# ShahzaibAhmad05/NextSearch-api

Measured on AMD Instinct MI355X. Metric: queries/sec at k=10 over 1M-doc index; achieved HBM GB/s vs peak, higher is better.
Workload: dtype f32

## Files before the change

nextsearch-api_amd/csrc/ns_api.hip:

```cpp
#include <hip/hip_runtime.h>

#include <algorithm>
#include <cmath>
#include <cstdarg>
#include <cstdio>
#include <cstdlib>
#include <cstring>
#include <string>
#include <vector>

#include "../../include/nextsearch_hip.h"
#include "ns_internal.h"
#include "ns_plan.hpp"
#include "ns_kernels.hip"
#include "ns_wave_kernel.hip"
#include "ns_driver_kernel.hip"
#include "ns_prune_kernel.hip"
#include "ns_merge_kernel.hip"
#include "ns_tile_kernel.hip"
#include "ns_invert.hip"
#include "ns_ingest.hip"
#include "ns_sem.hip"
#include "ns_suggest.hip"

// ... 1838 lines not shown
    ns_ctx* ctx = nullptr;
    uint32_t rows = 0, dim = 0, rows_pad = 0;
    float* d_vt = nullptr;
};

extern "C" int ns_sem_upload(ns_ctx* ctx, const float* vecs, uint32_t n_rows, uint32_t dim, ns_sem** out) {
    if (!ctx) return fail(nullptr, NS_E_INVAL, "ns_sem_upload: ctx is NULL");
    if (!out || !vecs || !n_rows || !dim) return fail(ctx, NS_E_INVAL, "ns_sem_upload: empty table or null argument");
    *out = nullptr;
    HIPCHK(ctx, hipSetDevice(ctx->device));
    ns_sem* s = new ns_sem();
    s->ctx = ctx; s->rows = n_rows; s->dim = dim; s->rows_pad = (n_rows + 63u) & ~63u;
    float* d_in = nullptr;
    hipError_t e = hipMalloc((void**)&s->d_vt, (size_t)dim * s->rows_pad * 4);
    if (e == hipSuccess) e = hipMalloc((void**)&d_in, (size_t)n_rows * dim * 4);
    if (e == hipSuccess) e = hipMemcpyAsync(d_in, vecs, (size_t)n_rows * dim * 4, hipMemcpyHostToDevice, ctx->stream);
    if (e == hipSuccess) {
        hipLaunchKernelGGL(k_sem_transpose, dim3((s->rows_pad + 31) / 32, (dim + 31) / 32), dim3(256), 0, ctx->stream, d_in, s->d_vt, n_rows, dim, s->rows_pad);
        e = hipGetLastError();
    }
    if (e == hipSuccess) e = hipStreamSynchronize(ctx->stream);
    (void)hipFree(d_in);
    if (e != hipSuccess) {
        (void)hipFree(s->d_vt);
        delete s;
        return fail(ctx, e == hipErrorOutOfMemory ? NS_E_NOMEM : NS_E_HIP, "ns_sem_upload: %s", hipGetErrorString(e));
    }
    *out = s;
    return NS_OK;
}

extern "C" int ns_sem_release(ns_ctx* ctx, ns_sem* sem) {
    if (!ctx || !sem || sem->ctx != ctx) return fail(ctx, NS_E_INVAL, "ns_sem_release: table does not belong to this ctx");
    HIPCHK(ctx, hipSetDevice(ctx->device));
    HIPCHK(ctx, hipStreamSynchronize(ctx->stream));
    (void)hipFree(sem->d_vt);
    delete sem;
    return NS_OK;
}

extern "C" int ns_sem_topk(ns_ctx* ctx, ns_sem* sem, const float* qvecs, uint32_t n_q, uint32_t topk, float min_sim,
                           const uint32_t* ban_off, const uint32_t* ban_rows, uint32_t* rows_out, float* sims_out,
                           uint32_t* counts_out, float* device_ms_out) {
    if (!ctx || !sem || sem->ctx != ctx) return fail(ctx, NS_E_INVAL, "ns_sem_topk: table does not belong to this ctx");
    if (topk < 1 || topk > (uint32_t)kSemMaxK) return fail(ctx, NS_E_INVAL, "ns_sem_topk: topk=%u outside [1,%d]", topk, kSemMaxK);
    if (device_ms_out) *device_ms_out = 0.0f;
    if (!n_q) return NS_OK;
    if (!qvecs || !rows_out || !sims_out || !counts_out) return fail(ctx, NS_E_INVAL, "ns_sem_topk: null argument");
    HIPCHK(ctx, hipSetDevice(ctx->device));
    hipStream_t st = ctx->stream;
    const uint32_t dim = sem->dim, rows = sem->rows, rp = sem->rows_pad;
    const uint32_t cap = ((rows + 63) / 64) * topk;
    const uint32_t n_groups = (n_q + kSemB - 1) / kSemB;
    const uint32_t n_ban = ban_off ? ban_off[n_q] : 0;
    std::vector<uint32_t> goff((size_t)n_groups * (kSemB + 1), 0), grows(std::max<uint32_t>(n_ban, 1), 0);
    if (n_ban && !ban_rows) return fail(ctx, NS_E_INVAL, "ns_sem_topk: ban_rows is NULL");
    if (n_ban) std::memcpy(grows.data(), ban_rows, (size_t)n_ban * 4);
    for (uint32_t g = 0; g < n_groups; g++)
        for (uint32_t b = 0; b <= (uint32_t)kSemB; b++) {
            const uint32_t qi = std::min(g * kSemB + b, n_q);
            goff[(size_t)g * (kSemB + 1) + b] = ban_off ? ban_off[qi] : 0;
        }
    std::vector<float> qpad((size_t)n_groups * kSemB * dim, 0.0f);
    std::memcpy(qpad.data(), qvecs, (size_t)n_q * dim * 4);

    float *d_q = nullptr, *d_osims = nullptr;
    uint32_t *d_goff = nullptr, *d_grows = nullptr, *d_orows = nullptr, *d_ocnt = nullptr, *d_count = nullptr;
    uint64_t* d_cand = nullptr;
    hipEvent_t ev0 = nullptr, ev1 = nullptr;
    hipError_t e = hipSuccess;
    auto chk = [&](hipError_t r) { if (e == hipSuccess) e = r; };
    const size_t n_pad = (size_t)n_groups * kSemB;
    size_t off = 0;
    auto place = [&](size_t bytes) { const size_t o = off; off = (off + std::max<size_t>(bytes, 1) + 255) & ~(size_t)255; return o; };
    const size_t o_q = place(qpad.size() * 4), o_cand = place((size_t)kSemB * cap * 8), o_goff = place(goff.size() * 4), o_count = place((size_t)kSemB * 4),
                 o_grows = place(grows.size() * 4), o_orows = place(n_pad * topk * 4), o_osims = place(n_pad * topk * 4), o_ocnt = place(n_pad * 4);
    const size_t block_bytes = off;
    char* blk = nullptr;
    chk(pool_alloc(ctx, (void**)&blk, block_bytes));
    if (e == hipSuccess) {
        d_q = (float*)(blk + o_q); d_cand = (uint64_t*)(blk + o_cand); d_goff = (uint32_t*)(blk + o_goff); d_count = (uint32_t*)(blk + o_count);
        d_grows = (uint32_t*)(blk + o_grows); d_orows = (uint32_t*)(blk + o_orows); d_osims = (float*)(blk + o_osims); d_ocnt = (uint32_t*)(blk + o_ocnt);
    }
    chk(hipEventCreate(&ev0));
    chk(hipEventCreate(&ev1));
    if (e == hipSuccess) {
        chk(hipMemcpyAsync(d_q, qpad.data(), qpad.size() * 4, hipMemcpyHostToDevice, st));
        chk(hipMemcpyAsync(d_goff, goff.data(), goff.size() * 4, hipMemcpyHostToDevice, st));
        chk(hipMemcpyAsync(d_grows, grows.data(), grows.size() * 4, hipMemcpyHostToDevice, st));
        chk(hipMemsetAsync(d_count, 0, (size_t)kSemB * 4, st));
        chk(hipEventRecord(ev0, st));
        for (uint32_t g = 0; g < n_groups; g++) {
            hipLaunchKernelGGL(k_sem_scan_topk, dim3((rows + 255) / 256), dim3(256), 0, st, sem->d_vt, rows, rp, dim, d_q + (size_t)g * kSemB * dim, min_sim,
                               d_goff + (size_t)g * (kSemB + 1), d_grows, topk, cap, d_cand, d_count);
            hipLaunchKernelGGL(k_sem_final_topk, dim3(kSemB), dim3(256), 0, st, d_cand, cap, d_count, topk, d_orows + (size_t)g * kSemB * topk, d_osims + (size_t)g * kSemB * topk, d_ocnt + (size_t)g * kSemB);
        }
        chk(hipEventRecord(ev1, st));
        chk(hipGetLastError());
        chk(hipMemcpyAsync(rows_out, d_orows, (size_t)n_q * topk * 4, hipMemcpyDeviceToHost, st));
        chk(hipMemcpyAsync(sims_out, d_osims, (size_t)n_q * topk * 4, hipMemcpyDeviceToHost, st));
        chk(hipMemcpyAsync(counts_out, d_ocnt, (size_t)n_q * 4, hipMemcpyDeviceToHost, st));
        chk(hipStreamSynchronize(st));
        float ms = 0.0f;
        if (e == hipSuccess && device_ms_out && hipEventElapsedTime(&ms, ev0, ev1) == hipSuccess) *device_ms_out = ms;
    }
    if (blk) { (void)hipStreamSynchronize(st); pool_free(ctx, blk, block_bytes); }
    if (ev0) (void)hipEventDestroy(ev0);
    if (ev1) (void)hipEventDestroy(ev1);
    if (e != hipSuccess) return fail(ctx, e == hipErrorOutOfMemory ? NS_E_NOMEM : NS_E_HIP, "ns_sem_topk: %s", hipGetErrorString(e));
    return NS_OK;
}

struct ns_ac {
    ns_ctx* ctx = nullptr;
    uint32_t n = 0;
    AcLevels lv{};
    uint8_t* d_pool = nullptr;
    uint32_t* d_offs = nullptr;
    uint64_t* d_heads = nullptr;
    uint64_t* d_keys = nullptr;
    uint64_t* d_tree = nullptr;
};

static void ac_free(ns_ac* ac) {
    if (!ac) return;
    (void)hipFree(ac->d_pool);
    (void)hipFree(ac->d_offs);
    (void)hipFree(ac->d_heads);
    (void)hipFree(ac->d_keys);
    (void)hipFree(ac->d_tree);
    delete ac;
}
static void ac_free_fwd(ns_ac* ac) { ac_free(ac); }

extern "C" int ns_ac_upload(ns_ctx* ctx, const uint8_t* pool, const uint64_t* offsets, const uint32_t* scores, uint32_t n_terms, ns_ac** out) {
    if (!ctx) return fail(nullptr, NS_E_INVAL, "ns_ac_upload: ctx is NULL");
    if (!out) return fail(ctx, NS_E_INVAL, "ns_ac_upload: out is NULL");
    *out = nullptr;
    if (n_terms && (!offsets || !scores)) return fail(ctx, NS_E_INVAL, "ns_ac_upload: null argument");
    if (n_terms == ~0u) return fail(ctx, NS_E_INVAL, "ns_ac_upload: %u terms (the index ~0 is reserved)", n_terms);
    const uint64_t pool_bytes = n_terms ? offsets[n_terms] : 0;
    if (n_terms && offsets[0] != 0) return fail(ctx, NS_E_INVAL, "ns_ac_upload: offsets[0] = %llu, not 0", (unsigned long long)offsets[0]);
    if (pool_bytes >= (1ull << 32)) return fail(ctx, NS_E_INVAL, "ns_ac_upload: a pool of %llu bytes (>= 4 GiB)", (unsigned long long)pool_bytes);
    if (pool_bytes && !pool) return fail(ctx, NS_E_INVAL, "ns_ac_upload: pool is NULL");
    for (uint32_t i = 0; i < n_terms; i++) {
        if (offsets[i + 1] < offsets[i]) return fail(ctx, NS_E_INVAL, "ns_ac_upload: offsets decrease at term %u", i);
        if (i == 0) continue;
        const uint64_t la = offsets[i] - offsets[i - 1], lb = offsets[i + 1] - offsets[i];
        const int c = std::memcmp(pool + offsets[i - 1], pool + offsets[i], (size_t)std::min(la, lb));
        if (c > 0 || (c == 0 && la > lb)) return fail(ctx, NS_E_INVAL, "ns_ac_upload: terms %u and %u are not in byte order", i - 1, i);
    }
    HIPCHK(ctx, hipSetDevice(ctx->device));
    ns_ac* ac = new ns_ac();
    ac->ctx = ctx;
    ac->n = n_terms;
    if (n_terms == 0) {
        ctx->acs.push_back(ac);
        *out = ac;
        return NS_OK;
    }
    std::vector<uint32_t> offs32(n_terms + 1);
    std::vector<uint64_t> heads(n_terms), keys(n_terms);
    for (uint32_t i = 0; i <= n_terms; i++) offs32[i] = (uint32_t)offsets[i];
    for (uint32_t i = 0; i < n_terms; i++) {
        const uint64_t len = offsets[i + 1] - offsets[i];
        uint64_t h = 0;
        for (uint64_t j = 0; j < len && j < 8; j++) h |= (uint64_t)pool[offsets[i] + j] << (56 - 8 * j);
        heads[i] = h;
        keys[i] = ((uint64_t)(~scores[i]) << 32) | i;
    }
    uint32_t nodes = (n_terms + kAcFan - 1) / kAcFan;
    uint64_t tree_keys = 0;
    for (;;) {
        ac->lv.off[ac->lv.n_levels] = tree_keys;
        ac->lv.nodes[ac->lv.n_levels] = nodes;
        tree_keys += (uint64_t)nodes * kAcTop;
        ac->lv.n_levels++;
        if (nodes <= (uint32_t)kAcFan) break;
        nodes = (nodes + kAcFan - 1) / kAcFan;
    }
    hipStream_t st = ctx->stream;
    hipError_t e = hipSuccess;
    auto chk = [&](hipError_t r) { if (e == hipSuccess) e = r; };
    chk(hipMalloc((void**)&ac->d_pool, std::max<uint64_t>(pool_bytes, 1)));
    chk(hipMalloc((void**)&ac->d_offs, (size_t)(n_terms + 1) * 4));
    chk(hipMalloc((void**)&ac->d_heads, (size_t)n_terms * 8));
    chk(hipMalloc((void**)&ac->d_keys, (size_t)n_terms * 8));
    chk(hipMalloc((void**)&ac->d_tree, (size_t)tree_keys * 8));
    if (e == hipSuccess) {
        if (pool_bytes) chk(hipMemcpyAsync(ac->d_pool, pool, pool_bytes, hipMemcpyHostToDevice, st));
        chk(hipMemcpyAsync(ac->d_offs, offs32.data(), offs32.size() * 4, hipMemcpyHostToDevice, st));
        chk(hipMemcpyAsync(ac->d_heads, heads.data(), heads.size() * 8, hipMemcpyHostToDevice, st));
        chk(hipMemcpyAsync(ac->d_keys, keys.data(), keys.size() * 8, hipMemcpyHostToDevice, st));
    }
    for (uint32_t j = 0; j < ac->lv.n_levels && e == hipSuccess; j++) {
        const uint64_t* src = j == 0 ? ac->d_keys : ac->d_tree + ac->lv.off[j - 1];
        const uint32_t n_src = j == 0 ? n_terms : ac->lv.nodes[j - 1];
        hipLaunchKernelGGL(k_ac_build, dim3((ac->lv.nodes[j] + 3) / 4), dim3(256), 0, st, src, n_src, j == 0 ? 1u : (uint32_t)kAcTop,
                           j == 0 ? 1u : (uint32_t)kAcTop, ac->d_tree + ac->lv.off[j], ac->lv.nodes[j]);
        chk(hipGetLastError());
    }
    chk(hipStreamSynchronize(st));
    if (e != hipSuccess) {
        ac_free(ac);
        return fail(ctx, e == hipErrorOutOfMemory ? NS_E_NOMEM : NS_E_HIP, "ns_ac_upload: %s", hipGetErrorString(e));
    }
    ctx->acs.push_back(ac);
    *out = ac;
    return NS_OK;
}

extern "C" int ns_ac_release(ns_ctx* ctx, ns_ac* ac) {
    if (!ctx) return fail(nullptr, NS_E_INVAL, "ns_ac_release: ctx is NULL");
    auto it = std::find(ctx->acs.begin(), ctx->acs.end(), ac);
    if (!ac || it == ctx->acs.end()) return fail(ctx, NS_E_INVAL, "ns_ac_release: table does not belong to this ctx");
    HIPCHK(ctx, hipSetDevice(ctx->device));
    HIPCHK(ctx, hipStreamSynchronize(ctx->stream));
    ctx->acs.erase(it);
    ac_free(ac);
    return NS_OK;
}

extern "C" int ns_ac_suggest(ns_ctx* ctx, ns_ac* ac, const uint8_t* prefix_bytes, const uint32_t* prefix_offsets, uint32_t n_q, uint32_t L,
                             uint32_t* idx_out, uint32_t* count_out, float* device_ms_out) {
    if (!ctx) return fail(nullptr, NS_E_INVAL, "ns_ac_suggest: ctx is NULL");
    if (!ac || std::find(ctx->acs.begin(), ctx->acs.end(), ac) == ctx->acs.end())
        return fail(ctx, NS_E_INVAL, "ns_ac_suggest: table does not belong to this ctx");
    if (L < 1 || L > (uint32_t)kAcTop) return fail(ctx, NS_E_INVAL, "ns_ac_suggest: L=%u outside [1,%d]", L, kAcTop);
    if (device_ms_out) *device_ms_out = 0.0f;
    if (!n_q) return NS_OK;
    if (!prefix_offsets || !idx_out || !count_out) return fail(ctx, NS_E_INVAL, "ns_ac_suggest: null argument");
    for (uint32_t q = 0; q < n_q; q++)
        if (prefix_offsets[q + 1] < prefix_offsets[q]) return fail(ctx, NS_E_INVAL, "ns_ac_suggest: prefix offsets decrease at %u", q);
    const uint32_t b0 = prefix_offsets[0], n_bytes = prefix_offsets[n_q] - b0;
    if (n_bytes && !prefix_bytes) return fail(ctx, NS_E_INVAL, "ns_ac_suggest: prefix_bytes is NULL");
    if (ac->n == 0) {
        std::fill(idx_out, idx_out + (size_t)n_q * L, ~0u);
        std::fill(count_out, count_out + n_q, 0u);
        return NS_OK;
    }
    HIPCHK(ctx, hipSetDevice(ctx->device));
    hipStream_t st = ctx->stream;
    const size_t o_bytes = ((size_t)(n_q + 1) * 4 + 7) & ~(size_t)7;
    const size_t up = o_bytes + n_bytes;
    const size_t o_idx = (up + 255) & ~(size_t)255;
    const size_t down = (size_t)n_q * L * 4 + (size_t)n_q * 4;
    const size_t block_bytes = o_idx + down;
    hipError_t e = hipSuccess;
    auto chk = [&](hipError_t r) { if (e == hipSuccess) e = r; };
    if (ctx->up_busy) {
        chk(hipEventSynchronize(ctx->up_done));
        ctx->up_busy = false;
    }
    if (e == hipSuccess && up <= kStageMaxBytes && ctx->h_up_cap < up) {
        if (ctx->h_up) (void)hipHostFree(ctx->h_up);
        ctx->h_up = nullptr; ctx->h_up_cap = 0;
        const size_t cap = std::max<size_t>(up + up / 2, 1 << 16);
        if (hipHostMalloc(&ctx->h_up, cap, hipHostMallocDefault) == hipSuccess) ctx->h_up_cap = cap;
        else { ctx->h_up = nullptr; (void)hipGetLastError(); }
    }
    const bool down_pinned = !ctx->down_owner && down <= kStageMaxBytes;
    if (e == hipSuccess && down_pinned && ctx->h_down_cap < down) {
        if (ctx->h_down) (void)hipHostFree(ctx->h_down);
        ctx->h_down = nullptr; ctx->h_down_cap = 0;
        const size_t cap = std::max<size_t>(down + down / 2, 1 << 16);
        if (hipHostMalloc(&ctx->h_down, cap, hipHostMallocDefault) == hipSuccess) ctx->h_down_cap = cap;
        else { ctx->h_down = nullptr; (void)hipGetLastError(); }
    }
    std::vector<char> up_own, down_own;
    char* hu = (ctx->h_up_cap >= up) ? (char*)ctx->h_up : (up_own.resize(up), up_own.data());
    char* hd = (down_pinned && ctx->h_down_cap >= down) ? (char*)ctx->h_down : (down_own.resize(down), down_own.data());
    for (uint32_t q = 0; q <= n_q; q++) ((uint32_t*)hu)[q] = prefix_offsets[q] - b0;
    if (n_bytes) std::memcpy(hu + o_bytes, prefix_bytes + b0, n_bytes);
    char* blk = nullptr;
    hipEvent_t ev0 = nullptr, ev1 = nullptr;
    if (e == hipSuccess) chk(pool_alloc(ctx, (void**)&blk, block_bytes));
    if (e == hipSuccess && device_ms_out) { chk(hipEventCreate(&ev0)); chk(hipEventCreate(&ev1)); }
    if (e == hipSuccess) {
        chk(hipMemcpyAsync(blk, hu, up, hipMemcpyHostToDevice, st));
        if (ev0) chk(hipEventRecord(ev0, st));
        hipLaunchKernelGGL(k_ac_suggest, dim3((n_q + 3) / 4), dim3(256), 0, st, ac->d_heads, ac->d_offs, ac->d_pool, ac->d_keys, ac->d_tree, ac->lv,
                           ac->n, (const uint8_t*)(blk + o_bytes), (const uint32_t*)blk, n_q, L, (uint32_t*)(blk + o_idx),
                           (uint32_t*)(blk + o_idx + (size_t)n_q * L * 4));
        chk(hipGetLastError());
        if (ev1) chk(hipEventRecord(ev1, st));
        chk(hipMemcpyAsync(hd, blk + o_idx, down, hipMemcpyDeviceToHost, st));
        chk(hipStreamSynchronize(st));
    }
    if (e == hipSuccess) {
        std::memcpy(idx_out, hd, (size_t)n_q * L * 4);
        std::memcpy(count_out, hd + (size_t)n_q * L * 4, (size_t)n_q * 4);
        float ms = 0.0f;
        if (ev0 && ev1 && hipEventElapsedTime(&ms, ev0, ev1) == hipSuccess) *device_ms_out = ms;
    }
    if (blk) { (void)hipStreamSynchronize(st); pool_free(ctx, blk, block_bytes); }
    if (ev0) (void)hipEventDestroy(ev0);
    if (ev1) (void)hipEventDestroy(ev1);
    if (e != hipSuccess) return fail(ctx, e == hipErrorOutOfMemory ? NS_E_NOMEM : NS_E_HIP, "ns_ac_suggest: %s", hipGetErrorString(e));
    return NS_OK;
}

#ifdef NS_COUNT
extern "C" int ns_debug_counters(unsigned long long* out, int reset) {
    unsigned long long h[20];
    if (hipDeviceSynchronize() != hipSuccess) return -1;
    if (hipMemcpyFromSymbol(h, HIP_SYMBOL(ns::g_ns_cnt), sizeof(h)) != hipSuccess) return -1;
    if (out) std::memcpy(out, h, sizeof(h));
    if (reset) { std::memset(h, 0, sizeof(h)); if (hipMemcpyToSymbol(HIP_SYMBOL(ns::g_ns_cnt), h, sizeof(h)) != hipSuccess) return -1; }
    return 0;
}
extern "C" int ns_debug_tile_counters(unsigned long long* out, int reset) {
    unsigned long long h[12];
    if (hipDeviceSynchronize() != hipSuccess) return -1;
    if (hipMemcpyFromSymbol(h, HIP_SYMBOL(ns::g_ns_tcnt), sizeof(h)) != hipSuccess) return -1;
    if (out) std::memcpy(out, h, sizeof(h));
    if (reset) { std::memset(h, 0, sizeof(h)); if (hipMemcpyToSymbol(HIP_SYMBOL(ns::g_ns_tcnt), h, sizeof(h)) != hipSuccess) return -1; }
    return 0;
}
#endif
```

nextsearch-api_amd/csrc/ns_driver_kernel.hip:

```cpp
#pragma once
#include <hip/hip_runtime.h>
#include <stdint.h>

#include "ns_internal.h"
#include "ns_wave_kernel.hip"

namespace ns {

#ifdef NS_COUNT
__device__ unsigned long long g_ns_cnt[20];
#define NS_CNT(i, v) cnt_[(i)] += (unsigned long long)(v)
#else
#define NS_CNT(i, v)
#endif

template <bool IMP, int PKM>
__device__ __forceinline__ void pk_decode_round(const DevSeg& seg, const uint32_t blk, const int lane, uint32_t (&doc)[4], float (&tf)[4],
                                                float (&nr)[4], uint32_t (&sbits)[4]) {
    const gp_u32 pb = (gp_u32)seg.packed + (size_t)blk * kPkStrideDwords + (uint32_t)lane;
    const uint32_t d0 = pb[kPkDoc], d1 = pb[kPkDoc + 64];
    uint32_t t = 0, na = 0, nb = 0;
    if (IMP) {
        const gp_f32 sc = (gp_f32)seg.pk_scores + (size_t)blk * kPkBlock + (uint32_t)lane;
#pragma unroll
        for (int c = 0; c < 4; c++) { sbits[c] = __float_as_uint(sc[c * 64]); tf[c] = 0.0f; nr[c] = 0.0f; }
    } else {
        t = pb[kPkTf];
        if (PKM == 2) { na = pb[kPkNormA]; nb = pb[kPkNormB]; }
        else {
            const gp_f32 np = (gp_f32)seg.pnorm + (size_t)blk * kPkBlock + (uint32_t)lane;
#pragma unroll
            for (int c = 0; c < 4; c++) nr[c] = np[c * 64];
        }
    }
    typedef const __attribute__((address_space(4))) uint32_t* cp_u32;
    const cp_u32 hp = (cp_u32)(const void*)(seg.pk_hdr + blk);
    const uint32_t base = hp[0];
    const uint32_t code = hp[1];
    if (code == 0u) {
#pragma unroll
        for (int c = 0; c < 4; c++) doc[c] = base + ((d0 >> (8 * c)) & 255u);
    } else if (code == 1u) {
        doc[0] = base + (d0 & 0xFFFFu); doc[1] = base + (d0 >> 16);
        doc[2] = base + (d1 & 0xFFFFu); doc[3] = base + (d1 >> 16);
    } else {
        doc[0] = d0; doc[1] = d1;
        doc[2] = pb[kPkDoc + 128]; doc[3] = pb[kPkDoc + 192];
    }
    if (!IMP) {
        uint32_t tfi[4];
#pragma unroll
        for (int c = 0; c < 4; c++) tfi[c] = (t >> (8 * c)) & 255u;
        const uint32_t nt_ = ~t;
        if (wballot(((nt_ - 0x01010101u) & t & 0x80808080u) != 0u) != 0ull) {
            const gp_u2 raw = (gp_u2)seg.postings + (size_t)blk * kPkBlock + (uint32_t)lane;
#pragma unroll
            for (int c = 0; c < 4; c++)
                if (tfi[c] == 255u) { const nat_u2 pv = raw[c * 64]; tfi[c] = pv.y; }
        }
        if (PKM == 2) {
            const gp_f32 ntab = (gp_f32)seg.ntab;
            nr[0] = ntab[na & 0xFFFFu]; nr[1] = ntab[na >> 16];
            nr[2] = ntab[nb & 0xFFFFu]; nr[3] = ntab[nb >> 16];
        }
#pragma unroll
        for (int c = 0; c < 4; c++) { tf[c] = (float)tfi[c]; sbits[c] = 0u; }
    }
}

__device__ __forceinline__ uint64_t lane_span(uint32_t lo, uint32_t hi) {
    const uint64_t upto_hi = hi >= 64u ? ~0ull : ((1ull << hi) - 1ull);
    const uint64_t upto_lo = lo >= 64u ? ~0ull : ((1ull << lo) - 1ull);
    return upto_hi & ~upto_lo;
}

template <int NB, int FB, bool AND, int CB = 256, bool IMP = false, int PK = 0>
__device__ __forceinline__ void dscore_body(const DevWItem& it, const DevTerm* __restrict__ terms, const DevSeg* __restrict__ segs,
                                            uint32_t* ent, float* vals, uint8_t* mcnt, uint64_t* cand, uint4* tab, uint32_t* aux,
                                            Hit* __restrict__ out_hits, uint32_t* __restrict__ out_nhits,
                                            uint64_t* __restrict__ out_found, uint32_t K, const int lane) {
    constexpr int FE = FB / 64;
    constexpr int DE = 4;
    constexpr uint32_t EMPTY = 0u;
    constexpr int LOG2NB = (NB == 64) ? 6 : (NB == 128 ? 7 : 8);
    constexpr uint32_t MAXSPAN = (1u << (LOG2NB + 15)) - 1u;
#define NS_BUCKET(doc) ((uint32_t)__builtin_amdgcn_ubfe(__umul24((doc) - lo, bm), 16u, (uint32_t)LOG2NB))
#define NS_TAG(doc) (0x8000u | (((doc) - lo) & 0x7FFFu))
#define NS_IDENT(doc, bkt) ((NS_TAG(doc) << 16) | ((bkt) << 8))
    static_assert(NB == 64 || NB == 128 || NB == 256, "NB must be 64, 128 or 256");
    static_assert(FB % 64 == 0 && FB >= 64 && FB <= 256 && FB <= 2 * NB, "FB must be a multiple of 64, at most 256 and 2*NB");
    uint4* ent4 = reinterpret_cast<uint4*>(ent);

#ifdef NS_COUNT
    const unsigned long long cyc_t0_ = __builtin_readcyclecounter();
#endif
    const DevSeg seg = segs[it.seg];
    const uint32_t T = it.term_count;
    const bool fast_div = (__builtin_amdgcn_readfirstlane((int)it.whole) & 8) != 0;
    const bool signed_in = (__builtin_amdgcn_readfirstlane((int)it.whole) & 16) != 0;
    const gp_u2 postings = (gp_u2)seg.postings;
    const gp_f32 pnorm = (gp_f32)seg.pnorm;
    const gp_u2 stream = IMP ? (gp_u2)seg.impacts : postings;

    {
        const uint4 empty4 = make_uint4(EMPTY, EMPTY, EMPTY, EMPTY);
#pragma unroll
        for (int g = 0; g < NB / 64; g++) ent4[g * 64 + lane] = empty4;
#pragma unroll
        for (int g = 0; g < FB / 64; g++) {
            vals[g * 64 + lane] = 0.0f;
            if (AND) mcnt[g * 64 + lane] = 0;
        }
    }

    uint32_t base = 0, cur = 0, end = 0, idf_bits = 0, wq_bits = 0;
    if ((uint32_t)lane < T) {
        const DevTerm tm = terms[it.term_begin + lane];
        base = (uint32_t)tm.list_off;
        idf_bits = __float_as_uint(tm.idf);
        wq_bits = __float_as_uint(tm.weight);
        const uint2 r = item_list_range(it, seg, tm);
        cur = r.x + base;
        end = r.y + base;
        tab[lane] = make_uint4(idf_bits, wq_bits, 0u, 0u);
    }
    uint32_t dl;
    {
        const uint32_t remv = end - cur;
        const uint32_t mx = wave_max_dpp(remv);
        dl = (uint32_t)__builtin_ctzll(wballot(remv == mx && (uint32_t)lane < T) | (1ull << 63));
        if (dl >= T) dl = 0;
    }
    uint32_t d_cur = rdlane(cur, dl);
    const uint32_t d_end = rdlane(end, dl);
    const float d_idf = __uint_as_float(rdlane(idf_bits, dl));
    const float d_wq = __uint_as_float(rdlane(wq_bits, dl));
    uint32_t Rf = 0;
    {
        const uint32_t r32 = ((uint32_t)lane == dl) ? 0u : (end - cur);
        for (uint32_t t = 0; t < T; t++) {
            const uint32_t v = rdlane(r32, t);
            Rf = (Rf + v < Rf) ? 0xFFFFFFFFu : (Rf + v);
        }
    }
    if ((uint32_t)lane == dl) { cur = end; }

#ifdef NS_COUNT
    unsigned long long cnt_[20] = {0, 0, 0, 0, 0, 0, 0, 0, 0, 0, 0, 0, 0, 0, 0, 0, 0, 0, 0, 0};
    cnt_[16] = __builtin_readcyclecounter() - cyc_t0_; cnt_[17] = 0;
    NS_CNT(0, 1);
    NS_CNT(10, T);
#endif
    uint32_t lo = it.doc_lo;
    const uint32_t last_doc = it.doc_hi - 1;
    WaveTopK<CB> top(cand, K, lane);
    uint32_t found_s = 0;

    uint32_t w_n = 0, e_n = 0xFFFFFFFFu;
#define NS_PLAN_FOREIGN()                                                                          \
    {                                                                                              \
        const uint32_t rem_ = end - cur;               \
        const uint32_t nact_ = (uint32_t)__popcll(wballot(rem_ > 0));                             \
        const float scale_ = (float)(FB - (int)nact_) * __builtin_amdgcn_rcpf((float)max(Rf, 1u)); \
        uint32_t w_ = 1u + (uint32_t)((float)rem_ * scale_);                                       \
        w_ = (w_ < rem_) ? w_ : rem_;                                                              \
        const bool probe_ = w_ < rem_;                                                             \
        const uint32_t pi_ = probe_ ? (cur + w_ - 1u) : 0u;                                        \
        const nat_u2 pv_ = postings[pi_];      \
        w_n = (rem_ > 0) ? w_ : 0u;                                                                \
        e_n = probe_ ? pv_.x : 0xFFFFFFFFu;                                                        \
    }
    NS_PLAN_FOREIGN();
    wave_sync();
    for (;;) {
        top.begin_step();
        NS_CNT(1, 1);
        const uint32_t w = w_n;
        const uint32_t e = e_n;
        const uint32_t incl = wave_incl_scan_dpp(w);
        const uint32_t total = rdlane(incl, 63);
        uint32_t hi = wave_min_dpp(e);
        const uint32_t span_hi = (last_doc - lo > MAXSPAN) ? (lo + MAXSPAN) : last_doc;
        const bool span_clamped = hi > span_hi && span_hi != last_doc;
        hi = min(hi, span_hi);
        uint32_t bm;
        {
            const uint32_t spn1 = (hi >= lo ? hi - lo : 0u) + 1u;
            bm = (uint32_t)((float)((uint32_t)NB << 16) * __builtin_amdgcn_rcpf((float)spn1));
            bm = (uint32_t)__builtin_amdgcn_readfirstlane((int)bm);
            while ((uint64_t)bm * spn1 > (uint64_t)((uint32_t)NB << 16)) bm--;
            while ((uint64_t)(bm + 1u) * spn1 <= (uint64_t)((uint32_t)NB << 16)) bm++;
            bm = min(bm, 0xFFFFFFu);
        }

        uint32_t ftj[FE];
        float fx[FE];
        bool fok[FE], fmine[FE];
        uint32_t fdoc[FE];
        uint32_t tb_min = 0, tb_max = 0;
#pragma unroll
        for (int j = 0; j < FE; j++) { ftj[j] = 0; fx[j] = 0.0f; fok[j] = false; fmine[j] = false; fdoc[j] = 0; }
        if (total > 0) {
            if ((uint32_t)lane < T) reinterpret_cast<uint2*>(tab + lane)[1] = make_uint2(cur - (incl - w), cur);
            if (T > 8 && (uint32_t)lane < T) aux[lane] = incl;
            wave_sync();
            if (T <= 8) {
                for (uint32_t t = 0; t + 1 < T; t++) {
                    const uint32_t sp = rdlane(incl, t);
#pragma unroll
                    for (int j = 0; j < FE; j++) ftj[j] += ((uint32_t)(j * 64 + lane) >= sp) ? 1u : 0u;
                }
            } else {
#pragma unroll
                for (int j = 0; j < FE; j++) {
                    const uint32_t p = min((uint32_t)(j * 64 + lane), total - 1u);
                    uint32_t a = 0, b = T - 1;
                    while (a < b) {
                        const uint32_t m = (a + b) >> 1;
                        if (aux[m] > p) b = m; else a = m + 1;
                    }
                    ftj[j] = a;
                }
                wave_sync();
            }
            nat_u2 pst[FE];
            float nrm[FE];
            uint32_t pidx[FE];
#pragma unroll
            for (int j = 0; j < FE; j++) {
                const uint32_t p = (uint32_t)(j * 64 + lane);
                const bool inb = p < total;
                ftj[j] = inb ? ftj[j] : 0u;
                pidx[j] = tab[ftj[j]].z + (inb ? p : 0u);
                pst[j] = stream[pidx[j]];
                nrm[j] = IMP ? 0.0f : pnorm[pidx[j]];
                pst[j].x = inb ? pst[j].x : 0xFFFFFFFFu;
            }
            uint32_t batch_consumed;
            {
                if ((uint32_t)lane < T) aux[lane] = cur + w;
                wave_sync();
                unsigned long long prev_last = 1ull;
#pragma unroll
                for (int j = 0; j < FE; j++) {
                    const bool take = pst[j].x <= hi;
                    fok[j] = take && (pst[j].x >= lo);
                    fdoc[j] = pst[j].x;
                    const unsigned long long m = wballot(take);
                    const bool prev_take = (((m << 1) | prev_last) >> lane) & 1ull;
                    prev_last = m >> 63;
                    const bool first_untaken = ((uint32_t)(j * 64 + lane) < total) && !take &&
                                               (prev_take || pidx[j] == tab[ftj[j]].w);
                    if (first_untaken) aux[ftj[j]] = pidx[j];
                }
                wave_sync();
                uint32_t c = 0;
                if ((uint32_t)lane < T && (uint32_t)lane != dl) {
                    const uint32_t ncur = aux[lane];
                    c = ncur - cur;
                    cur = ncur;
                }
                c += dpp_mov<0x111, 0xf>(0u, c);
                c += dpp_mov<0x112, 0xf>(0u, c);
                c += dpp_mov<0x114, 0xf>(0u, c);
                c += dpp_mov<0x118, 0xf>(0u, c);
                c += dpp_mov<0x142, 0xa>(0u, c);
                c += dpp_mov<0x143, 0xc>(0u, c);
                batch_consumed = rdlane(c, 63);
            }
            if (batch_consumed == 0 && !span_clamped) {
                if ((uint32_t)lane != dl) { cur += w; if (cur > end) cur = end; }
                batch_consumed = total;
            }
            NS_CNT(2, 1);
            NS_CNT(3, total);
            NS_CNT(4, batch_consumed);
            NS_CNT(5, (total + 63) / 64);
            NS_CNT(11, (uint32_t)__popcll(wballot(w > 0)));
            Rf = (Rf > batch_consumed) ? (Rf - batch_consumed) : 0;
            NS_PLAN_FOREIGN();
            tb_min = rdlane(ftj[0], 0);
            {
                const uint32_t lastp = total - 1u;
                uint32_t tl = 0;
#pragma unroll
                for (int j = 0; j < FE; j++)
                    if ((lastp >> 6) == (uint32_t)j) tl = rdlane(ftj[j], lastp & 63u);
                tb_max = tl;
            }
            {
                float num[FE], den[FE], wqv[FE];
#pragma unroll
                for (int j = 0; j < FE; j++) {
                    const uint4 te = tab[ftj[j]];
                    const float tf = (float)pst[j].y;
                    den[j] = tf + nrm[j];
                    num[j] = __uint_as_float(te.x) * (tf * (1.2f + 1.0f));
                    wqv[j] = __uint_as_float(te.y);
                }
                if (IMP) {
#pragma unroll
                    for (int j = 0; j < FE; j++) fx[j] = __uint_as_float(pst[j].y);
                } else {
                    ns_div_n<FE>(fx, num, den, fast_div);
                }
#pragma unroll
                for (int j = 0; j < FE; j++) fx[j] = wqv[j] * fx[j];
            }
            uint32_t pterm = 0xFFFFFFFFu;
            {
                const uint32_t wmax = wave_max_dpp(w);
                if (wmax >= 8u) pterm = (uint32_t)__builtin_ctzll(wballot(w == wmax));
            }
            if (pterm != 0xFFFFFFFFu) {
                uint32_t carry_b = 0xFFFFFFFFu, carry_n = 0u;
                bool sorted_ok = true;
#pragma unroll
                for (int j = 0; j < FE; j++) {
                    const bool isp = fok[j] && ftj[j] == pterm;
                    const uint64_t pm = wballot(isp);
                    if ((uint32_t)(j * 64) < total && pm != 0ull && sorted_ok) {
                        const uint32_t bkt = NS_BUCKET(fdoc[j]);
                        const uint32_t bprev = (uint32_t)__builtin_amdgcn_ds_bpermute((lane - 1) << 2, (int)bkt);
                        const bool prevp = __builtin_amdgcn_inverse_ballot_w64(pm << 1);
                        sorted_ok = wballot(isp && prevp && bkt < bprev) == 0ull &&
                                    (carry_b == 0xFFFFFFFFu || rdlane(bkt, (uint32_t)__builtin_ctzll(pm)) >= carry_b);
                        if (sorted_ok) {
                            uint32_t hl = (isp && (!prevp || bkt != bprev)) ? (uint32_t)lane : 0u;
                            hl = max(hl, dpp_mov<0x111, 0xf>(0u, hl));
                            hl = max(hl, dpp_mov<0x112, 0xf>(0u, hl));
                            hl = max(hl, dpp_mov<0x114, 0xf>(0u, hl));
                            hl = max(hl, dpp_mov<0x118, 0xf>(0u, hl));
                            hl = max(hl, dpp_mov<0x142, 0xa>(0u, hl));
                            hl = max(hl, dpp_mov<0x143, 0xc>(0u, hl));
                            const uint32_t pos = ((bkt == carry_b) ? carry_n : 0u) + ((uint32_t)lane - hl);
                            const uint32_t at = bkt * 4u + pos;
                            if (isp && pos < 4u) {
                                ent[at] = NS_IDENT(fdoc[j], bkt) | (uint32_t)(j * 64 + lane);
                                fmine[j] = true;
                                ftj[j] |= ((uint32_t)(j * 64 + lane) << 6) | (at << 14);
                            }
                            const uint32_t last = 63u - (uint32_t)__builtin_clzll(pm);
                            carry_b = rdlane(bkt, last);
                            carry_n = rdlane(pos, last) + 1u;
                            NS_CNT(15, (uint32_t)__popcll(wballot(isp && pos < 4u)));
                        }
                    }
                }
                wave_sync();
            }
#pragma unroll
            for (int j = 0; j < FE; j++) {
                if ((uint32_t)(j * 64) >= total) continue;
                bool pending = fok[j] && !fmine[j];
                if (wballot(pending) == 0ull) continue;
                const uint32_t me = (uint32_t)(j * 64 + lane);
                uint32_t b = NS_BUCKET(fdoc[j]);
                const uint32_t mine = NS_IDENT(fdoc[j], b) | me;
                const bool todo = pending;
                uint32_t slot = 0, own = 0;
                bool scan = pending;
                uint32_t pos = 0;
                for (int round = 0; round < 8 * NB; round++) {
                    if (wballot(pending) == 0ull) break;
                    NS_CNT(6, 1);
                    if (wballot(scan) != 0ull) {
                        if (scan) {
                            const uint4 q = ent4[b];
                            const uint32_t tmin = min(min(q.x ^ mine, q.y ^ mine), min(q.z ^ mine, q.w ^ mine));
                            pos = (q.x >> 31) + (q.y >> 31) + (q.z >> 31) + (q.w >> 31);
                            if (tmin < 256u) { own = tmin ^ me; pending = false; }
                            scan = false;
                        }
                    }
                    const bool try_store = pending && pos < 4;
                    if (try_store) ent[b * 4 + pos] = mine;
                    wave_sync();
                    if (try_store) {
                        const uint32_t back = ent[b * 4 + pos];
                        if ((back ^ mine) < 256u) { slot = b * 4 + pos; own = back & 255u; pending = false; }
                        else pos++;
                    } else if (pending) {
                        b = (b + 1) & (uint32_t)(NB - 1);
                        scan = true;
                    }
                    wave_sync();
                }
                if (todo) {
                    fmine[j] = own == me;
                    ftj[j] |= (own << 6) | (slot << 14);
                }
            }
        }

#define NS_FOREIGN_RMW(ta, tb)                                                                     \
        for (uint32_t tt = (ta); tt <= (tb); tt++) {                                               \
            if (tt == dl) continue;                                                                \
            NS_CNT(7, 1);                                                                          \
            float old_[FE];                                                                        \
             \
                                    \
            _Pragma("unroll") for (int j = 0; j < FE; j++) {                                       \
                const bool c_ = fok[j] && (ftj[j] & 63u) == tt;                                    \
                old_[j] = vals[c_ ? ((ftj[j] >> 6) & 255u) : (uint32_t)(j * 64 + lane)];           \
            }                                                                                      \
            _Pragma("unroll") for (int j = 0; j < FE; j++) {                                       \
                if (fok[j] && (ftj[j] & 63u) == tt) {                                              \
                    const uint32_t o_ = (ftj[j] >> 6) & 255u;                                      \
                    vals[o_] = old_[j] + fx[j];                                                    \
                    if (AND) mcnt[o_] = (uint8_t)(mcnt[o_] + 1);                                   \
                }                                                                                  \
            }                                                                                      \
            wave_sync();                                                                           \
        }
        if (total > 0 && tb_min < dl) { NS_FOREIGN_RMW(tb_min, min(tb_max, dl - 1)); }

        bool driver_progress = false;
        for (;;) {
            const uint32_t remd = d_end - d_cur;
            if (remd == 0) break;
            uint32_t n;
            nat_u2 ps[DE];
            float nr[DE];
            float tfv[DE];
            uint32_t sbits[DE];
            uint32_t cnt = 0, r_hits = 0;
            NS_CNT(8, 1);
            float dx[DE];
            uint64_t dokm[DE];
            uint32_t first_pos, last_pos;
            if (PK) {
                static_assert(DE == 4, "a packed round is one block of 4 chunks");
                const uint32_t blk = d_cur >> 8;
                const uint32_t a = d_cur & 255u;
                const uint32_t e = min(256u, d_end - (blk << 8));
                n = e - a;
                first_pos = a; last_pos = e - 1u;
                uint32_t docs_[4];
                pk_decode_round<IMP, PK>(seg, blk, lane, docs_, tfv, nr, sbits);
#pragma unroll
                for (int j = 0; j < DE; j++) { ps[j].x = docs_[j]; ps[j].y = sbits[j]; }
                if (n == (uint32_t)(DE * 64)) {
#pragma unroll
                    for (int j = 0; j < DE; j++) {
                        dokm[j] = wballot(ps[j].x <= hi);
                        cnt += (uint32_t)__popcll(dokm[j]);
                    }
                } else {
#pragma unroll
                    for (int j = 0; j < DE; j++) {
                        const uint32_t c0 = (uint32_t)(j * 64);
                        const uint64_t vm = lane_span(a > c0 ? a - c0 : 0u, e > c0 ? min(e - c0, 64u) : 0u);
                        dokm[j] = wballot(ps[j].x <= hi) & vm;
                        cnt += (uint32_t)__popcll(dokm[j]);
                    }
                }
            } else {
                n = min(remd, (uint32_t)(DE * 64));
                first_pos = 0u; last_pos = n - 1u;
                const gp_u2 sp = stream + d_cur;
                const gp_f32 np = pnorm + d_cur;
#pragma unroll
                for (int j = 0; j < DE; j++) {
                    ps[j] = sp[j * 64 + lane];
                    nr[j] = IMP ? 0.0f : np[j * 64 + lane];
                    tfv[j] = (float)ps[j].y;
                }
                if (n == (uint32_t)(DE * 64)) {
#pragma unroll
                    for (int j = 0; j < DE; j++) {
                        dokm[j] = wballot(ps[j].x <= hi);
                        cnt += (uint32_t)__popcll(dokm[j]);
                    }
                } else {
#pragma unroll
                    for (int j = 0; j < DE; j++) {
                        const uint32_t left = (n > (uint32_t)(j * 64)) ? (n - (uint32_t)(j * 64)) : 0u;
                        const uint64_t nmask = (left >= 64u) ? ~0ull : ((1ull << left) - 1ull);
                        dokm[j] = wballot(ps[j].x <= hi) & nmask;
                        cnt += (uint32_t)__popcll(dokm[j]);
                    }
                }
            }
            NS_CNT(12, (n + 63) / 64);
            {
                float num[DE], den[DE];
#pragma unroll
                for (int j = 0; j < DE; j++) {
                    const float tf = tfv[j];
                    den[j] = tf + nr[j];
                    num[j] = d_idf * (tf * (1.2f + 1.0f));
                }
                if (IMP) {
#pragma unroll
                    for (int j = 0; j < DE; j++) dx[j] = __uint_as_float(ps[j].y);
                } else {
                    ns_div_n<DE>(dx, num, den, fast_div);
                }
#pragma unroll
                for (int j = 0; j < DE; j++) dx[j] = d_wq * dx[j];
                if (signed_in) {
#pragma unroll
                    for (int j = 0; j < DE; j++) dx[j] = 0.0f + dx[j];
                }
            }
            bool any_foreign_here = total > 0;
            if (FB <= 64 && total > 0) {
                uint32_t rfirst, rlast;
                if (n == (uint32_t)(DE * 64)) {
                    rfirst = rdlane(ps[0].x, 0);
                    rlast = rdlane(ps[DE - 1].x, 63);
                } else {
                    rfirst = 0; rlast = 0;
#pragma unroll
                    for (int j = 0; j < DE; j++) {
                        if ((first_pos >> 6) == (uint32_t)j) rfirst = rdlane(ps[j].x, first_pos & 63u);
                        if ((last_pos >> 6) == (uint32_t)j) rlast = rdlane(ps[j].x, last_pos & 63u);
                    }
                }
                bool here = false;
#pragma unroll
                for (int j = 0; j < FE; j++) here = here || (fok[j] && fdoc[j] >= rfirst && fdoc[j] <= rlast);
                any_foreign_here = wballot(here) != 0ull;
            }
            if (any_foreign_here) {
#pragma unroll
                for (int j = 0; j < DE; j++) {
                    if (dokm[j] == 0ull) continue;
                    const uint32_t tag = NS_TAG(ps[j].x);
                    const uint32_t hb = NS_BUCKET(ps[j].x);
                    uint32_t b = hb;
                    uint4 q = ent4[b];
                    const uint64_t cm = wballot((q.x >> 16) == tag) | wballot((q.y >> 16) == tag) |
                                        wballot((q.z >> 16) == tag) | wballot((q.w >> 16) == tag);
                    const uint64_t go = dokm[j] & (cm | wballot(q.w != EMPTY));
                    if (go != 0ull) {
                        const uint32_t ident = NS_IDENT(ps[j].x, hb);
                        uint32_t m = 0;
                        bool more = __builtin_amdgcn_inverse_ballot_w64(go);
                        while (wballot(more) != 0ull) {
                            if (more) {
                                m = ((q.x ^ ident) < 256u) ? q.x : m;
                                m = ((q.y ^ ident) < 256u) ? q.y : m;
                                m = ((q.z ^ ident) < 256u) ? q.z : m;
                                m = ((q.w ^ ident) < 256u) ? q.w : m;
                                more = m == 0 && q.w != EMPTY;
                                if (more) { b = (b + 1) & (uint32_t)(NB - 1); q = ent4[b]; }
                            }
                        }
                        const uint64_t hitm = wballot(m != 0);
                        if (hitm != 0ull) {
                            if (m != 0) {
                                const uint32_t o = m & 255u;
                                vals[o] = vals[o] + dx[j];
                                if (AND) mcnt[o] = (uint8_t)(mcnt[o] + 1);
                            }
                            dokm[j] &= ~hitm;
                            r_hits += (uint32_t)__popcll(hitm);
                        }
                    }
                }
            }
            if (!AND || T == 1) {
                found_s += cnt - r_hits;
#pragma unroll
                for (int j = 0; j < DE; j++) {
                    top.offer_mask_stream(dokm[j], dx[j], ps[j].x);
                }
            }
            NS_CNT(9, cnt);
            NS_CNT(13, any_foreign_here ? (n + 63) / 64 : 0);
            NS_CNT(14, r_hits);
            d_cur += cnt;
            driver_progress = driver_progress || (cnt > 0);
            if (cnt < n) break;
        }

        if (total > 0) {
            if (tb_max > dl) { NS_FOREIGN_RMW(max(tb_min, dl + 1), tb_max); }
            float fin[FE];
            bool scored[FE];
#pragma unroll
            for (int j = 0; j < FE; j++) {
                fin[j] = vals[j * 64 + lane];
                scored[j] = fmine[j];
                if (AND && fmine[j]) scored[j] = (mcnt[j * 64 + lane] == (uint8_t)T);
            }
            wave_sync();
#pragma unroll
            for (int j = 0; j < FE; j++) {
                vals[j * 64 + lane] = 0.0f;
                if (fmine[j]) {
                    ent[ftj[j] >> 14] = EMPTY;
                    if (AND) mcnt[j * 64 + lane] = 0;
                }
                found_s += (uint32_t)__popcll(wballot(scored[j]));
                top.offer(scored[j], fin[j], fdoc[j]);
            }
            wave_sync();
        }
        top.keep_room();

        if (hi >= last_doc) break;
        if (Rf == 0 && d_cur >= d_end) break;
        if (total == 0 && !driver_progress) break;
        lo = hi + 1;
    }
#undef NS_FOREIGN_RMW
#undef NS_PLAN_FOREIGN
#undef NS_TAG
#undef NS_IDENT
#undef NS_BUCKET

#ifdef NS_COUNT
    const unsigned long long cyc_t1_ = __builtin_readcyclecounter();
#endif
    top.write_out(it.seg, it.out_slot, found_s, out_hits, out_nhits, out_found);
#ifdef NS_COUNT
    cnt_[17] = __builtin_readcyclecounter() - cyc_t0_;
    cnt_[18] = __builtin_readcyclecounter() - cyc_t1_;
    if (lane == 0)
        for (int i = 0; i < 20; i++) if (cnt_[i]) atomicAdd(&g_ns_cnt[i], cnt_[i]);
#endif
}

template <int HK, int FB, bool AND>
__global__ void __launch_bounds__(256) k_dscore(const DevWItem* __restrict__ items, uint32_t n_items,
                                                const DevTerm* __restrict__ terms, const DevSeg* __restrict__ segs,
                                                Hit* __restrict__ out_hits, uint32_t* __restrict__ out_nhits,
                                                uint64_t* __restrict__ out_found, uint32_t K) {
    constexpr int WPB = 4;
    __shared__ __attribute__((aligned(16))) uint32_t s_ent[WPB][HK];
    __shared__ __attribute__((aligned(16))) float s_vals[WPB][FB];
    __shared__ __attribute__((aligned(16))) uint8_t s_mcnt[WPB][AND ? FB : 16];
    __shared__ uint64_t s_cand[WPB][256];
    __shared__ __attribute__((aligned(16))) uint4 s_tab[WPB][64];
    __shared__ uint32_t s_aux[WPB][64];
    const int wave = __builtin_amdgcn_readfirstlane((int)(threadIdx.x >> 6));
    const int lane = threadIdx.x & 63;
    const uint32_t item_idx = blockIdx.x * WPB + wave;
    if (item_idx >= n_items) return;
    const DevWItem it = items[item_idx];
    dscore_body<HK / 4, FB, AND>(it, terms, segs, s_ent[wave], s_vals[wave], s_mcnt[wave], s_cand[wave], s_tab[wave], s_aux[wave],
                                 out_hits, out_nhits, out_found, K, lane);
}

}
```

Before: 7.763 million.

## Extend sorted-run fast placement to all terms with bounded per-term steps

The fast hash-slot placement that used to cover only the single largest term (when it had at least 8 postings) now runs for every foreign term. Entries are keyed by term and offset, checked for sortedness, and placed in up to 8 per-term rounds that look up existing bucket entries to join or append. The fmine flags are dropped and recomputed from the ownership bits packed into ftj, which removes register state. The aim is to send fewer entries through the slower scan-based fallback placement, at the cost of extra ballots, LDS reads and wave syncs per round.

```diff
diff --git a/nextsearch-api_amd/csrc/ns_api.hip b/nextsearch-api_amd/csrc/ns_api.hip
--- a/nextsearch-api_amd/csrc/ns_api.hip
+++ b/nextsearch-api_amd/csrc/ns_api.hip
@@ -2164,7 +2164,7 @@
 
 #ifdef NS_COUNT
 extern "C" int ns_debug_counters(unsigned long long* out, int reset) {
-    unsigned long long h[20];
+    unsigned long long h[24];
     if (hipDeviceSynchronize() != hipSuccess) return -1;
     if (hipMemcpyFromSymbol(h, HIP_SYMBOL(ns::g_ns_cnt), sizeof(h)) != hipSuccess) return -1;
     if (out) std::memcpy(out, h, sizeof(h));
diff --git a/nextsearch-api_amd/csrc/ns_driver_kernel.hip b/nextsearch-api_amd/csrc/ns_driver_kernel.hip
--- a/nextsearch-api_amd/csrc/ns_driver_kernel.hip
+++ b/nextsearch-api_amd/csrc/ns_driver_kernel.hip
@@ -8,7 +8,7 @@
 namespace ns {
 
 #ifdef NS_COUNT
-__device__ unsigned long long g_ns_cnt[20];
+__device__ unsigned long long g_ns_cnt[24];
 #define NS_CNT(i, v) cnt_[(i)] += (unsigned long long)(v)
 #else
 #define NS_CNT(i, v)
@@ -84,7 +84,8 @@
     constexpr uint32_t EMPTY = 0u;
     constexpr int LOG2NB = (NB == 64) ? 6 : (NB == 128 ? 7 : 8);
     constexpr uint32_t MAXSPAN = (1u << (LOG2NB + 15)) - 1u;
-#define NS_BUCKET(doc) ((uint32_t)__builtin_amdgcn_ubfe(__umul24((doc) - lo, bm), 16u, (uint32_t)LOG2NB))
+#define NS_BUCKET_OFF(off) ((uint32_t)__builtin_amdgcn_ubfe(__umul24((off), bm), 16u, (uint32_t)LOG2NB))
+#define NS_BUCKET(doc) NS_BUCKET_OFF((doc) - lo)
 #define NS_TAG(doc) (0x8000u | (((doc) - lo) & 0x7FFFu))
 #define NS_IDENT(doc, bkt) ((NS_TAG(doc) << 16) | ((bkt) << 8))
     static_assert(NB == 64 || NB == 128 || NB == 256, "NB must be 64, 128 or 256");
@@ -146,7 +147,7 @@
     if ((uint32_t)lane == dl) { cur = end; }
 
 #ifdef NS_COUNT
-    unsigned long long cnt_[20] = {0, 0, 0, 0, 0, 0, 0, 0, 0, 0, 0, 0, 0, 0, 0, 0, 0, 0, 0, 0};
+    unsigned long long cnt_[24] = {};
     cnt_[16] = __builtin_readcyclecounter() - cyc_t0_; cnt_[17] = 0;
     NS_CNT(0, 1);
     NS_CNT(10, T);
@@ -195,11 +196,11 @@
 
         uint32_t ftj[FE];
         float fx[FE];
-        bool fok[FE], fmine[FE];
+        bool fok[FE];
         uint32_t fdoc[FE];
         uint32_t tb_min = 0, tb_max = 0;
 #pragma unroll
-        for (int j = 0; j < FE; j++) { ftj[j] = 0; fx[j] = 0.0f; fok[j] = false; fmine[j] = false; fdoc[j] = 0; }
+        for (int j = 0; j < FE; j++) { ftj[j] = 0; fx[j] = 0.0f; fok[j] = false; fdoc[j] = 0; }
         if (total > 0) {
             if ((uint32_t)lane < T) reinterpret_cast<uint2*>(tab + lane)[1] = make_uint2(cur - (incl - w), cur);
             if (T > 8 && (uint32_t)lane < T) aux[lane] = incl;
@@ -307,56 +308,83 @@
 #pragma unroll
                 for (int j = 0; j < FE; j++) fx[j] = wqv[j] * fx[j];
             }
-            uint32_t pterm = 0xFFFFFFFFu;
+            constexpr int kPlaceSteps = 8;
+            uint64_t pendm[FE];
+            bool sorted_ok = true;
             {
-                const uint32_t wmax = wave_max_dpp(w);
-                if (wmax >= 8u) pterm = (uint32_t)__builtin_ctzll(wballot(w == wmax));
-            }
-            if (pterm != 0xFFFFFFFFu) {
-                uint32_t carry_b = 0xFFFFFFFFu, carry_n = 0u;
-                bool sorted_ok = true;
 #pragma unroll
                 for (int j = 0; j < FE; j++) {
-                    const bool isp = fok[j] && ftj[j] == pterm;
-                    const uint64_t pm = wballot(isp);
-                    if ((uint32_t)(j * 64) < total && pm != 0ull && sorted_ok) {
-                        const uint32_t bkt = NS_BUCKET(fdoc[j]);
-                        const uint32_t bprev = (uint32_t)__builtin_amdgcn_ds_bpermute((lane - 1) << 2, (int)bkt);
-                        const bool prevp = __builtin_amdgcn_inverse_ballot_w64(pm << 1);
-                        sorted_ok = wballot(isp && prevp && bkt < bprev) == 0ull &&
-                                    (carry_b == 0xFFFFFFFFu || rdlane(bkt, (uint32_t)__builtin_ctzll(pm)) >= carry_b);
-                        if (sorted_ok) {
-                            uint32_t hl = (isp && (!prevp || bkt != bprev)) ? (uint32_t)lane : 0u;
-                            hl = max(hl, dpp_mov<0x111, 0xf>(0u, hl));
-                            hl = max(hl, dpp_mov<0x112, 0xf>(0u, hl));
-                            hl = max(hl, dpp_mov<0x114, 0xf>(0u, hl));
-                            hl = max(hl, dpp_mov<0x118, 0xf>(0u, hl));
-                            hl = max(hl, dpp_mov<0x142, 0xa>(0u, hl));
-                            hl = max(hl, dpp_mov<0x143, 0xc>(0u, hl));
-                            const uint32_t pos = ((bkt == carry_b) ? carry_n : 0u) + ((uint32_t)lane - hl);
-                            const uint32_t at = bkt * 4u + pos;
-                            if (isp && pos < 4u) {
-                                ent[at] = NS_IDENT(fdoc[j], bkt) | (uint32_t)(j * 64 + lane);
-                                fmine[j] = true;
-                                ftj[j] |= ((uint32_t)(j * 64 + lane) << 6) | (at << 14);
-                            }
-                            const uint32_t last = 63u - (uint32_t)__builtin_clzll(pm);
-                            carry_b = rdlane(bkt, last);
-                            carry_n = rdlane(pos, last) + 1u;
-                            NS_CNT(15, (uint32_t)__popcll(wballot(isp && pos < 4u)));
+                    pendm[j] = wballot(fok[j]);
+                    if ((uint32_t)(j * 64) >= total || pendm[j] == 0ull || !sorted_ok) continue;
+                    uint32_t mine, hl;
+                    {
+                        const uint32_t key = (ftj[j] << 24) | ((fdoc[j] - lo) & 0xFFFFFFu);
+                        const uint32_t kprev = (uint32_t)__builtin_amdgcn_ds_bpermute((lane - 1) << 2, (int)key);
+                        const bool prevl = __builtin_amdgcn_inverse_ballot_w64(pendm[j] << 1);
+                        const bool same_term = lane != 0 && ((kprev ^ key) >> 24) == 0u;
+                        sorted_ok = wballot(fok[j] && same_term && (!prevl || kprev >= key)) == 0ull;
+                        if (!sorted_ok) continue;
+                        const uint32_t bkt = NS_BUCKET_OFF(key);
+                        const uint32_t bprev = NS_BUCKET_OFF(kprev);
+                        mine = NS_IDENT(fdoc[j], bkt);
+                        asm volatile("" : "+v"(mine));
+                        mine |= (uint32_t)(j * 64 + lane);
+                        hl = (fok[j] && !(prevl && same_term && bprev == bkt)) ? (uint32_t)lane : 0u;
+                        hl = max(hl, dpp_mov<0x111, 0xf>(0u, hl));
+                        hl = max(hl, dpp_mov<0x112, 0xf>(0u, hl));
+                        hl = max(hl, dpp_mov<0x114, 0xf>(0u, hl));
+                        hl = max(hl, dpp_mov<0x118, 0xf>(0u, hl));
+                        hl = max(hl, dpp_mov<0x142, 0xa>(0u, hl));
+                        hl = max(hl, dpp_mov<0x143, 0xc>(0u, hl));
+                    }
+                    uint64_t rem = pendm[j];
+                    for (int step = 0; step < kPlaceSteps && rem != 0ull; step++) {
+                        NS_CNT(19, 1);
+                        const uint32_t t = rdlane(ftj[j], (uint32_t)__builtin_ctzll(rem)) & 63u;
+                        const bool act = fok[j] && (ftj[j] & 63u) == t;
+                        rem &= ~wballot(act);
+                        const uint32_t bkt = (mine >> 8) & 255u;
+                        const uint4 q = ent4[bkt];
+                        const uint32_t tmin = min(min(q.x ^ mine, q.y ^ mine), min(q.z ^ mine, q.w ^ mine));
+                        const uint32_t fill = (q.x >> 31) + (q.y >> 31) + (q.z >> 31) + (q.w >> 31);
+                        const bool join = act && tmin < 256u;
+                        const uint64_t sm = wballot(act && tmin >= 256u);
+                        const uint32_t below = lanes_below(sm);
+                        const uint32_t pos = fill + (below - (uint32_t)__builtin_amdgcn_ds_bpermute((int)(hl << 2), (int)below));
+                        const uint32_t at = bkt * 4u + pos;
+                        const bool put = act && tmin >= 256u && pos < 4u;
+                        if (put) {
+                            ent[at] = mine;
+                            ftj[j] |= ((mine & 255u) << 6) | (at << 14);
                         }
-                    }
-                }
-                wave_sync();
-            }
+                        if (join) ftj[j] |= ((tmin ^ mine) & 255u) << 6;
+                        const uint64_t putm = wballot(put);
+                        pendm[j] &= ~(putm | wballot(join));
+                        NS_CNT(15, (uint32_t)__popcll(putm));
+                        wave_sync();
+                    }
+                }
+            }
+#ifdef NS_COUNT
+            {
+                uint32_t nfb = 0;
+#pragma unroll
+                for (int j = 0; j < FE; j++) nfb += (uint32_t)__popcll(pendm[j]);
+                NS_CNT(20, nfb);
+                NS_CNT(21, nfb != 0 ? 1 : 0);
+                NS_CNT(22, sorted_ok ? 0 : 1);
+            }
+#endif
 #pragma unroll
             for (int j = 0; j < FE; j++) {
                 if ((uint32_t)(j * 64) >= total) continue;
-                bool pending = fok[j] && !fmine[j];
-                if (wballot(pending) == 0ull) continue;
+                if (pendm[j] == 0ull) continue;
+                bool pending = __builtin_amdgcn_inverse_ballot_w64(pendm[j]);
                 const uint32_t me = (uint32_t)(j * 64 + lane);
                 uint32_t b = NS_BUCKET(fdoc[j]);
-                const uint32_t mine = NS_IDENT(fdoc[j], b) | me;
+                uint32_t mine = NS_IDENT(fdoc[j], b);
+                asm volatile("" : "+v"(mine));
+                mine |= me;
                 const bool todo = pending;
                 uint32_t slot = 0, own = 0;
                 bool scan = pending;
@@ -386,10 +414,7 @@
                     }
                     wave_sync();
                 }
-                if (todo) {
-                    fmine[j] = own == me;
-                    ftj[j] |= (own << 6) | (slot << 14);
-                }
+                if (todo) ftj[j] |= (own << 6) | (slot << 14);
             }
         }
 
@@ -578,19 +603,20 @@
 
         if (total > 0) {
             if (tb_max > dl) { NS_FOREIGN_RMW(max(tb_min, dl + 1), tb_max); }
+#define NS_FMINE(j) (fok[j] && ((ftj[j] >> 6) & 255u) == (uint32_t)((j) * 64 + lane))
             float fin[FE];
             bool scored[FE];
 #pragma unroll
             for (int j = 0; j < FE; j++) {
                 fin[j] = vals[j * 64 + lane];
-                scored[j] = fmine[j];
-                if (AND && fmine[j]) scored[j] = (mcnt[j * 64 + lane] == (uint8_t)T);
+                scored[j] = NS_FMINE(j);
+                if (AND && scored[j]) scored[j] = (mcnt[j * 64 + lane] == (uint8_t)T);
             }
             wave_sync();
 #pragma unroll
             for (int j = 0; j < FE; j++) {
                 vals[j * 64 + lane] = 0.0f;
-                if (fmine[j]) {
+                if (NS_FMINE(j)) {
                     ent[ftj[j] >> 14] = EMPTY;
                     if (AND) mcnt[j * 64 + lane] = 0;
                 }
@@ -606,11 +632,13 @@
         if (total == 0 && !driver_progress) break;
         lo = hi + 1;
     }
+#undef NS_FMINE
 #undef NS_FOREIGN_RMW
 #undef NS_PLAN_FOREIGN
 #undef NS_TAG
 #undef NS_IDENT
 #undef NS_BUCKET
+#undef NS_BUCKET_OFF
 
 #ifdef NS_COUNT
     const unsigned long long cyc_t1_ = __builtin_readcyclecounter();
@@ -620,7 +648,7 @@
     cnt_[17] = __builtin_readcyclecounter() - cyc_t0_;
     cnt_[18] = __builtin_readcyclecounter() - cyc_t1_;
     if (lane == 0)
-        for (int i = 0; i < 20; i++) if (cnt_[i]) atomicAdd(&g_ns_cnt[i], cnt_[i]);
+        for (int i = 0; i < 24; i++) if (cnt_[i]) atomicAdd(&g_ns_cnt[i], cnt_[i]);
 #endif
 }
 
```

After: 7.714 million. About the same (-0.6%).
